# Thealexbarney/VGAudio

Measured on AMD Instinct MI355X. Metric: Msamples/s encoded (GC-ADPCM, 4096 ch) at 1/2/4/8 GPUs; % HBM roofline, higher is better.
Workload: dtype int32; 1 GPU; BASELINE configs[1]: 4096 mono channels x 48 kHz x 60 s GC-ADPCM coefficient search + encode per GPU; parallelism=units sharded x1, channels_per_gpu=4096, samples_per_channel=2880000, bit_exact_channels_checked=0

## Files before the change

vgaudio_amd/csrc/capi_gcadpcm.hip:

```cpp
#include "gc_capi.hpp"
#include "../../include/vgaudio_hip_testing.h"

using namespace vga;

extern "C" {

int vga_testing_gc_plan_pieces(int cus, int groups, int frames, long long group_frames, int ragged, int *out5)
{
    if (!out5 || cus <= 0 || groups <= 0 || frames <= 0) return -1;
    bool persistent = false;
    gc::Pieces seg;
    const int segments = gc::plan_encode_pieces_on(cus, groups, frames, group_frames, ragged != 0, &persistent, &seg);
    out5[0] = segments;
    out5[1] = seg.big;
    out5[2] = seg.nb;
    out5[3] = seg.small;
    out5[4] = persistent ? 1 : 0;
    return 0;
}

int vga_gcadpcm_nibble_count_to_sample_count(int nibble_count) { return gc::nibble_count_to_sample_count(nibble_count); }
int vga_gcadpcm_sample_count_to_nibble_count(int sample_count) { return gc::sample_count_to_nibble_count(sample_count); }
int vga_gcadpcm_nibble_to_sample(int nibble) { return gc::nibble_to_sample(nibble); }
int vga_gcadpcm_sample_to_nibble(int sample) { return gc::sample_to_nibble(sample); }
int vga_gcadpcm_sample_count_to_byte_count(int sample_count) { return gc::sample_count_to_byte_count(sample_count); }
int vga_gcadpcm_byte_count_to_sample_count(int byte_count) { return gc::byte_count_to_sample_count(byte_count); }

size_t vga_gcadpcm_coefs_workspace_bytes(int nch, int length)
{
    if (nch <= 0 || length < 0) return 0;
    const size_t frames = ((size_t)length + 13) / 14;
    return (size_t)nch * (size_t)vga::gc::coef_record_pitch((int64_t)frames) * 16;
}

int vga_gcadpcm_coefs_device(const int16_t *d_pcm, int64_t pcm_pitch, int nch, int length, int16_t *d_coefs,
// ... 287 lines not shown
```

vgaudio_amd/csrc/gc_capi.hpp:

```cpp
#pragma once
#include "common.hpp"
#include "host_batch.hpp"
#include "gcadpcm_kernels.hpp"
#include "gc_host.hpp"

#include <cstring>
#include <vector>

namespace vga {
namespace gc {

constexpr int GC_MIN_SHARE_CHANNELS = 128;

struct GcBatch {
    Stream st;
    DevBuf pcm, coefs, adpcm, h1, h2, ws, status;
    int64_t pcm_pitch = 0, adpcm_pitch = 0;
};

inline int upload_hist(DevBuf &d_h1, DevBuf &d_h2, int nch, const int16_t *h1, const int16_t *h2, const Stream *async_on)
{
    DevBuf *const dst[2] = {&d_h1, &d_h2};
    const int16_t *const src[2] = {h1, h2};
    for (int k = 0; k < 2; k++) {
// ... 13 lines not shown
    int64_t records = 0;
    Pieces seg;
    int segments = 1;
    bool persistent = false;
    std::vector<uint32_t> items;

    void build(const int *lengths, int n, int64_t pcm_base, int64_t adpcm_base)
    {
        lay_out(lengths, n, pcm_base, adpcm_base);
        rec_off.resize(n);
        records = 0;
        for (int c = 0; c < n; c++) {
            rec_off[c] = records;
            records += coef_record_pitch(((int64_t)length[c] + 13) / 14);
        }
        items.clear();
        solo_channels = solo_usable = 0;
        if (n > 0 && !uniform && max_length > 0) {
            std::vector<int> by_length(n);
            for (int i = 0; i < n; i++) by_length[i] = length[order[i]];
            solo_channels = ragged_solo_count(by_length.data(), n, total_frames, device_cu_count(), &solo_usable);
            const int groups = (int)group_frames.size();
            const int64_t work = std::accumulate(group_frames.begin(), group_frames.end(), (int64_t)0);
            segments = plan_encode_pieces(groups, (max_length + 13) / 14, work, true, &persistent, &seg);
            if (persistent && groups < (1 << 20) && segments <= 4096) {
                struct Item { int size, y, g; };
                std::vector<Item> list;
                for (int y = 0; y < segments; y++)
                    for (int g = 0; g < groups; g++)
                        if (seg.first(y) < group_frames[g])
                            list.push_back({(int)std::min<int64_t>(seg.frames(y), group_frames[g] - seg.first(y)), y, g});
                std::stable_sort(list.begin(), list.end(), [](const Item &a, const Item &b) { return a.size > b.size; });
                items.reserve(list.size());
                for (const Item &it : list) items.push_back(((uint32_t)it.y << 20) | (uint32_t)it.g);
            } else
                persistent = false;
        }
    }
    size_t table_bytes() const { return (size_t)round_up((int64_t)count * 8, 16) + (size_t)count * 24 + items.size() * 4; }
    void write_tables(unsigned char *host) const
    {
        int *o = reinterpret_cast<int *>(host);
        int *l = o + count;
        int64_t *p = reinterpret_cast<int64_t *>(host + round_up((int64_t)count * 8, 16));
        for (int c = 0; c < count; c++) {
            o[c] = order[c];
            l[c] = length[c];
// ... 58 lines not shown
```

vgaudio_amd/csrc/gc_encode_kernel.hip:

```cpp
#include "common.hpp"
#include "gc_encode_core.hpp"
#include "gcadpcm_kernels.hpp"
#include "seams.hpp"

#include <cstdio>
#include <cstdlib>

namespace vga {
namespace gc {

constexpr int DPP_QUAD_XOR1 = 0xB1;
constexpr int DPP_QUAD_XOR2 = 0x4E;
constexpr int DPP_ROW_HALF_MIRROR = 0x141;
constexpr int DPP_ROW_MIRROR = 0x140;

template <int CTRL>
__device__ __forceinline__ int dpp(int v)
{
    return __builtin_amdgcn_update_dpp(0, v, CTRL, 0xF, 0xF, true);
}

__device__ __forceinline__ unsigned umin32(unsigned a, unsigned b) { return a < b ? a : b; }

template <class Op>
__device__ __forceinline__ unsigned row16_reduce(unsigned v, Op op)
{
// ... 19 lines not shown
    if (out8 && hipMemcpyFromSymbol(out8, HIP_SYMBOL(g_vga_gc_stats), 8 * sizeof(unsigned long long)) != hipSuccess) return -1;
#ifdef VGA_GC_STATS
    if (out8) out8[7] = 1;
#else
    if (out8) out8[7] = 0;
#endif
    if (reset) {
        const unsigned long long zero[8] = {0, 0, 0, 0, 0, 0, 0, 0};
        if (hipMemcpyToSymbol(HIP_SYMBOL(g_vga_gc_stats), zero, sizeof zero) != hipSuccess) return -1;
    }
    return 0;
}
constexpr int SW = 2;
constexpr int ENC_THREADS = 64 * (SW + 1);
#ifndef VGA_GC_ENCODER_PRIO
#define VGA_GC_ENCODER_PRIO 3
#endif
#ifndef VGA_GC_HELPER_PRIO
#define VGA_GC_HELPER_PRIO 0
#endif
#ifndef VGA_GC_PERSISTENT_WAVES_PER_EU
#define VGA_GC_PERSISTENT_WAVES_PER_EU 3, 3
#endif
template <int CPW>
struct Lay {
    static constexpr int CS = CPW * SW;
    static constexpr int TF = 64 / CS;
};
template <int CS, int TF>
struct GcTileT {
    struct Slot {
        uint32_t xw[8];
        int in2048p[16];
        uint32_t pre[8];
        int4 out[4];
    };
    struct Group { Slot f[TF]; uint32_t pad[4]; };
    Group g[CS];
};
typedef short short2v __attribute__((ext_vector_type(2)));
struct XW7 { uint32_t v[7]; };

#define VGA_COLD __device__ __forceinline__

VGA_COLD int prescan_sequential_cold(XW7 xs, uint32_t hist, int c0, int c1)
{
    int x[16];
    unpack_row(xs.v, hist, x);
    return prescan_sequential(x, c0, c1);
}
// ... 56 lines not shown
                if ((unsigned)r.max_overflow > (cap ? 3u : 248u)) {
                    int xg[16];
                    unpack_row(xw, st.hist, xg);
#pragma unroll
                    for (int i = 0; i < 16; i++) VGA_COLD_OPAQUE(xg[i]);
                    r = as_pass_b(resume_passes(xg, st.c0, st.c1, sp - 1, final_sp));
                    sum_exact = 1;
                    break;
                }
                final_sp = sp;
                if (cap || r.max_overflow <= 1) break;
            }
            fin = 1;
        }
    }
    ColdOut o;
    o.r = r;
    o.final_sp = final_sp;
    o.fin = fin;
    o.sum_exact = sum_exact;
    return o;
}

template <bool REPAIR, int CPW, bool RAGGED>
__device__ __forceinline__ void gc_encode_piece(
    const int bx, const int by,
    const int16_t *__restrict__ pcm, int64_t pcm_pitch, int nch, int total_samples, const Pieces seg,
    const int16_t *__restrict__ coefs, const int16_t *__restrict__ hist1,
    const int16_t *__restrict__ hist2, uint8_t *__restrict__ adpcm, int64_t adpcm_pitch, int16_t *__restrict__ seg_state,
    const int *__restrict__ first_open, const Ragged &rg)
{
    constexpr bool repair = REPAIR;
    constexpr int CS = Lay<CPW>::CS, TF = Lay<CPW>::TF;
    using GcTile = GcTileT<CS, TF>;
    int64_t first_frame = seg.first(by);
    int repair_piece = 0;
    if (repair) {
        int k = SEAM_OPEN_LIMIT;
        for (int g = 0; g < CS; g++) {
            const int slot = bx * CS + g;
            if (slot < nch) {
                const int c = RAGGED ? rg.order[slot] : slot;
                k = first_open[c] < k ? first_open[c] : k;
            }
        }
        if (!is_open(k)) return;
        repair_piece = k;
        first_frame = seg.first(k);
    }
    const int total_wg = RAGGED ? rg.length[rg.order[bx * CS]] : total_samples;
    if (first_frame * 14 >= total_wg) return;
    const int64_t piece_samples = repair ? (int64_t)0x7fffffff : (int64_t)seg.frames(by) * 14;
    auto piece_samples_of = [&](int total) {
        const int64_t rem = (int64_t)total - first_frame * 14;
        return (int)(rem < 0 ? 0 : (rem < piece_samples ? rem : piece_samples));
    };
    pcm += first_frame * 14;
    adpcm += first_frame * 8;
    using Slot = typename GcTile::Slot;
    static_assert(TF % 2 == 0, "the frame loop takes a tile's frames in pairs");
    struct Tiles { GcTile t[2]; Slot end; };
    __shared__ Tiles s_tiles;
    GcTile (&s_tile)[2] = s_tiles.t;
    __shared__ int s_ncold[SW];
    const int tid = threadIdx.x;
    const int wave = tid >> 6;
    const bool helper = wave == SW;
    const int lane = tid & 63;
    constexpr int LPC = 64 / CPW;
    int grp = helper ? lane / TF : wave * CPW + lane / LPC;
    const int l16 = lane & (LPC - 1);
    const int hfr = lane % TF;
    const int slot_raw = bx * CS + grp;
    const bool live = slot_raw < nch;
    const int slot = live ? slot_raw : nch - 1;
    const int ch = RAGGED ? rg.order[slot] : slot;
    const int16_t *src = pcm + (RAGGED ? rg.pcm_off[ch] : (int64_t)ch * pcm_pitch);
    uint8_t *dst = adpcm + (RAGGED ? rg.adpcm_off[ch] : (int64_t)ch * adpcm_pitch);

    const int sample_count = piece_samples_of(RAGGED ? rg.length[ch] : total_samples);
    const int full_frames = sample_count / 14;
    const int tail = sample_count - full_frames * 14;
    const int frames = full_frames + (tail ? 1 : 0);
    const int frames_wg = RAGGED ? (piece_samples_of(total_wg) + 13) / 14 : frames;
    const int tiles = (frames_wg + TF - 1) / TF;

    if (helper) {
        __builtin_amdgcn_s_setprio(VGA_GC_HELPER_PRIO);
        uint32_t cpk[8];
#pragma unroll
        for (int p = 0; p < 8; p++)
            cpk[p] = (uint32_t)(uint16_t)coefs[ch * 16 + 2 * p + 1] | ((uint32_t)(uint16_t)coefs[ch * 16 + 2 * p] << 16);
        auto prepare = [&](int tile) {
            const int fr = RAGGED ? imax(imin(tile * TF + hfr, frames - 1), 0) : imin(tile * TF + hfr, frames - 1);
            int in[14];
            uint32_t w[7];
            if (fr < full_frames) {
                const uint32_t *p32 = reinterpret_cast<const uint32_t *>(src + (int64_t)fr * 14);
#pragma unroll
                for (int i = 0; i < 7; i++) w[i] = p32[i];
#pragma unroll
                for (int i = 0; i < 7; i++) {
                    in[2 * i] = (int)(int16_t)(w[i] & 0xFFFF);
                    in[2 * i + 1] = (int)w[i] >> 16;
                }
            } else {
#pragma unroll
                for (int s = 0; s < 14; s++) in[s] = (s < tail) ? (int)src[(int64_t)fr * 14 + s] : 0;
#pragma unroll
                for (int i = 0; i < 7; i++) w[i] = (uint32_t)(in[2 * i] & 0xFFFF) | ((uint32_t)in[2 * i + 1] << 16);
            }
            Slot &T = s_tile[tile & 1].g[grp].f[hfr];
            uint4 *xr = reinterpret_cast<uint4 *>(&T.xw[0]);
            xr[0] = make_uint4(w[0], w[1], w[2], w[3]);
            xr[1] = make_uint4(w[4], w[5], w[6], (!RAGGED || tile * TF + hfr < frames) ? 1u : 0u);
            int4 *qr = reinterpret_cast<int4 *>(&T.in2048p[0]);
            qr[0] = make_int4(pass_b_row(in[0]), pass_b_row(in[1]), pass_b_row(in[2]), pass_b_row(in[3]));
            qr[1] = make_int4(pass_b_row(in[4]), pass_b_row(in[5]), pass_b_row(in[6]), pass_b_row(in[7]));
            qr[2] = make_int4(pass_b_row(in[8]), pass_b_row(in[9]), pass_b_row(in[10]), pass_b_row(in[11]));
            qr[3] = make_int4(pass_b_row(in[12]), pass_b_row(in[13]), 0, 0);
            uint32_t pair[12];
#pragma unroll
            for (int k = 0; k < 12; k++)
                pair[k] = (k & 1) ? __builtin_amdgcn_alignbit(w[(k + 1) / 2], w[(k - 1) / 2], 16) : w[k / 2];
            uint32_t pre[8];
#pragma unroll
            for (int p = 0; p < 8; p++) {
                int dmax = 0, dmin = 0;
#ifdef VGA_GC_ABLATE_HELPER_PRESCAN
                dmax = in[2 + p] & 1023;
                dmin = -(in[3 + p] & 1023);
#else
#pragma unroll
                for (int k = 0; k < 12; k++) {
                    const int predicted = div2048(__builtin_amdgcn_sdot2(__builtin_bit_cast(short2v, pair[k]),
                                                                         __builtin_bit_cast(short2v, cpk[p]), 0, false));
                    const int d = in[k + 2] - predicted;
                    dmax = imax(dmax, d);
                    dmin = imin(dmin, d);
                }
#endif
                pre[p] = (uint32_t)(clamp16i(dmax) & 0xFFFF) | ((uint32_t)clamp16i(dmin) << 16);
            }
            uint4 *pr = reinterpret_cast<uint4 *>(&T.pre[0]);
            pr[0] = make_uint4(pre[0], pre[1], pre[2], pre[3]);
            pr[1] = make_uint4(pre[4], pre[5], pre[6], pre[7]);
        };
        auto flush = [&](int tile) {
            const int fr = tile * TF + hfr;
            if (!live || fr >= frames) return;
            const int4 *rec = &s_tile[tile & 1].g[grp].f[hfr].out[0];
            const int4 r0 = rec[0], r1 = rec[1], r2 = rec[2], r3 = rec[3];
            const int q[14] = {r0.x, r0.y, r0.z, r0.w, r1.x, r1.y, r1.z, r1.w, r2.x, r2.y, r2.z, r2.w, r3.x, r3.y};
            uint2 v;
            pack_frame_mod16(q, r3.z, r3.w, v.x, v.y);
            if (fr < full_frames) {
                *reinterpret_cast<uint2 *>(dst + (int64_t)fr * 8) = v;
            } else {
                const int nbytes = (tail + 2 + 1) / 2;
                const uint64_t both = ((uint64_t)v.y << 32) | v.x;
                for (int b = 0; b < nbytes; b++) dst[(int64_t)fr * 8 + b] = (uint8_t)(both >> (8 * b));
            }
        };
        if (tiles > 0) prepare(0);
        __syncthreads();
        for (int tile = 0; tile < tiles; tile++) {
            if (tile + 1 < tiles) prepare(tile + 1);
            if (tile > 0) flush(tile - 1);
            __syncthreads();
        }
        if (tiles > 0) flush(tiles - 1);
        return;
    }

    __builtin_amdgcn_s_setprio(VGA_GC_ENCODER_PRIO);
    const int wave_u = __builtin_amdgcn_readfirstlane(wave);
    int p = CPW == 4 ? l16 >> 1 : l16;
    const bool cand_b = CPW == 4 && (l16 & 1) != 0;
    const int c0 = coefs[ch * 16 + 2 * p];
    const int c1 = coefs[ch * 16 + 2 * p + 1];
    const bool coef_ok = pass_b_coef_ok(c0, c1);
    int h0 = hist2 ? hist2[ch] : 0;
    int h1 = hist1 ? hist1[ch] : 0;
    if (repair) {
        h0 = seg_state[((int64_t)(repair_piece - 1) * nch + ch) * 2];
        h1 = seg_state[((int64_t)(repair_piece - 1) * nch + ch) * 2 + 1];
    } else if (by > 0 && (!RAGGED || frames > 0)) {
        h0 = src[-2];
        h1 = src[-1];
    }
    uint32_t hpk = pack16(h0, h1);

    if (lane == 0) s_ncold[wave] = 0;
    struct Row { uint32_t xw[7]; int mp[14]; };
    auto read_row = [&](const Slot &T, Row &R) {
        const uint4 *xr = reinterpret_cast<const uint4 *>(&T.xw[0]);
        const uint4 a0 = xr[0], a1 = xr[1];
        asm volatile("" ::"v"(a1.w));
// ... 236 lines not shown
#endif
            st.bump_a = bump_a; st.ov_a = ov_a; st.ov_b = ov_2;
            const ColdOut o = encode_frame_cold(st, r, final_sp, (generic || resume) ? 0 : 1);
            bool sat2 = false;
            int winner = argmin32(o.r, o.fin != 0, sat2);
            if (sat2) {
                uint64_t total = o.r.total;
                if (o.fin != 0 && needs_exact_sum(total, o.sum_exact != 0))
                    total = wide_total(xw, R.mp, o.final_sp);
                winner = argmin64(total, o.fin != 0);
            }
            commit(o.r, o.final_sp, winner);
        } else
            commit(r, final_sp, winner32);
    };
    auto encode_one = [&](Row &R, Slot &S, uint32_t pre) __attribute__((always_inline)) {
        if constexpr (CPW == 4) encode_frame(R, S, pre);
        else encode_frame8(R, S, pre);
    };

#ifdef VGA_DEBUG_TIMESTAMPS
    if (!repair && tid == 0 && gridDim.y != 1) g_vga_enc_ts[2 * ((blockIdx.y * gridDim.x + blockIdx.x) & 32767)] = wall_clock64();
#endif
    __syncthreads();
    for (int tile = 0; tile < tiles; tile++) {
        const int buf = tile & 1;
        const int nf = imin(TF, frames_wg - tile * TF);
#ifndef VGA_GC_NO_TILE_REDERIVE
        {
            unsigned zero = 0;
            asm volatile("" : "+s"(zero));
            const int l = (int)__builtin_amdgcn_mbcnt_hi(~0u, __builtin_amdgcn_mbcnt_lo(~0u, zero));
            grp = wave_u * CPW + l / LPC;
            p = CPW == 4 ? (l & (LPC - 1)) >> 1 : (l & (LPC - 1));
        }
#endif
        Slot *S = &s_tile[buf].g[grp].f[0];
        Row RA, RB;
        read_row(S[0], RA);
#pragma unroll 1
        for (int j = 0; j < nf; j += 2, S += 2) {
            const uint32_t pre_a = read_pre(S[0]);
            read_row(S[1], RB);
            encode_one(RA, S[0], pre_a);
            if (j + 1 < nf) {
                const uint32_t pre_b = read_pre(S[1]);
                read_row(S[2], RA);
                encode_one(RB, S[1], pre_b);
            }
        }
        __syncthreads();
    }
    if (seg_state && !repair && live && l16 == 0) {
        int16_t *st = seg_state + ((int64_t)by * nch + ch) * 2;
        st[0] = (int16_t)pair_lo(hpk);
        st[1] = (int16_t)pair_hi(hpk);
    }
    if (lane == 0) {
        atomicAdd(&g_vga_gc_stats[3], (unsigned long long)frames_wg);
        atomicAdd(&g_vga_gc_stats[4], (unsigned long long)s_ncold[wave]);
        if (wave == 0) atomicAdd(&g_vga_gc_stats[6], 1ull);
    }
#ifdef VGA_DEBUG_TIMESTAMPS
    if (!repair && tid == 0 && gridDim.y != 1) g_vga_enc_ts[2 * ((blockIdx.y * gridDim.x + blockIdx.x) & 32767) + 1] = wall_clock64();
#endif
}


template <bool REPAIR, int CPW, bool RAGGED>
__global__ __launch_bounds__(ENC_THREADS) __attribute__((amdgpu_waves_per_eu(3, 3))) void gc_encode_kernel(
    const int16_t *__restrict__ pcm, int64_t pcm_pitch, int nch, int total_samples, const Pieces seg,
    const int16_t *__restrict__ coefs, const int16_t *__restrict__ hist1,
    const int16_t *__restrict__ hist2, uint8_t *__restrict__ adpcm, int64_t adpcm_pitch, int16_t *__restrict__ seg_state,
    const int *__restrict__ first_open, const Ragged rg)
// ... 302 lines not shown
            auto exists = [&](int piece) { return piece < segments && seg.first(piece) * 14 < total_wg; };
            int at_start = 0, at_end = 0;
            if (exists(y)) {
                if (y >= 1 && atomicAdd(&seam_count[(int64_t)(y - 1) * groups + g], 1) == 1) at_start = y;
                if (exists(y + 1) && atomicAdd(&seam_count[(int64_t)y * groups + g], 1) == 1) at_end = y + 1;
            }
            s_seam[0] = at_start;
            s_seam[1] = at_end;
        }
        __syncthreads();
        const int seam_a = s_seam[0], seam_b = s_seam[1];
        if ((seam_a | seam_b) != 0) {
            __threadfence();
            const int wave = threadIdx.x >> 6, lane = threadIdx.x & 63;
            if (wave < SW) {
                const int slot = g * CS + wave * CPW + (lane >> 3);
                if (seam_a)
                    seam_piece<8>(slot, seam_a, lane, pcm, pcm_pitch, nch, total_samples, seg, coefs, adpcm, adpcm_pitch, seg_state,
                               first_open, seam_flag, seam_end, force_open, rg);
                if (seam_b)
                    seam_piece<8>(slot, seam_b, lane, pcm, pcm_pitch, nch, total_samples, seg, coefs, adpcm, adpcm_pitch, seg_state,
                               first_open, seam_flag, seam_end, force_open, rg);
            }
        }
    }
}

template <int LPC>
__global__ __launch_bounds__(64) void gc_encode_chain_kernel(
    const int16_t *__restrict__ pcm, int64_t pcm_pitch, int nch, int total_samples, const Pieces seg, int segments,
    const int16_t *__restrict__ coefs, uint8_t *__restrict__ adpcm, int64_t adpcm_pitch,
    int16_t *__restrict__ seg_state, int *__restrict__ first_open, const int *__restrict__ seam_flag,
    const int *__restrict__ seam_end, int force_open, const Ragged rg)
{
    const int lane = threadIdx.x;
    const int pr = LPC == 16 ? (lane >> 1) & 7 : lane & 7;
    const bool lead = (lane & (LPC - 1)) == 0;
    const int slot_raw = blockIdx.x * (64 / LPC) + lane / LPC;
    const bool live = slot_raw < nch;
    const int slot = live ? slot_raw : nch - 1;
    const int ch = rg.order ? rg.order[slot] : slot;
    if (rg.order) total_samples = rg.length[ch];
    const int mine = live ? first_open[ch] : SEAM_NONE;
    int kmin = mine;
#pragma unroll
    for (int o = LPC; o < 64; o <<= 1) kmin = imin(kmin, __shfl_xor(kmin, o));
// ... 35 lines not shown
        } else if (flagged) {
            have = true;
            v0 = (int)(int16_t)(ended & 0xFFFF);
            v1 = ended >> 16;
        } else
            have = false;
    }
    if (__any(live && have && total_samples % 14 != 0))
        encode_tail_frame<LPC>(src, dst, c0, c1, coef_ok, pr, total_samples, v0, v1, live && have && total_samples % 14 != 0);
    (void)last_k;
    if (live && lead && frames_run) atomicAdd(&g_vga_gc_stats[2], (unsigned long long)frames_run);
    if (live && lead) first_open[ch] = SEAM_NONE;
}

constexpr int MIN_PIECE_FRAMES = 3584;

constexpr int RAGGED_OVERSUBSCRIPTION = 4;
constexpr int PERSISTENT_MIN_GROUPS_FACTOR = 32;
constexpr int PERSISTENT_SCHEDULE_GROUPS_FACTOR = 8;
constexpr int PERSISTENT_ITEMS_PER_WORKGROUP = 4;
constexpr int PERSISTENT_BIG_ROUNDS = 3;
constexpr int PERSISTENT_SMALL_ROUNDS = 2;
constexpr int PERSISTENT_SMALL_FRAMES = 4096;
constexpr int MAX_PIECES = 1024;

static int persistent_wgs_per_cu()
{
#ifdef VGA_TUNING
    if (const char *e = std::getenv("VGA_HIP_GC_WGS_PER_CU")) return imin(imax(std::atoi(e), 1), 5);
#endif
    return 4;
}

int plan_encode_pieces(int groups, int frames, int64_t group_frames, bool ragged, bool *persistent_out, Pieces *seg_out, int layout)
{
    return plan_encode_pieces_on(device_cu_count(), groups, frames, group_frames, ragged, persistent_out, seg_out, layout);
}

int plan_encode_pieces_on(int cus, int groups, int frames, int64_t group_frames, bool ragged, bool *persistent_out, Pieces *seg_out, int layout)
{
    const int pmode = encoder_persistent_mode();
    const bool persistent = layout != 4 && (pmode == 2 || (pmode == 0 && (ragged || groups * PERSISTENT_MIN_GROUPS_FACTOR >= cus * 4)));
    int segments = cus * 4 / (groups > 0 ? groups : 1);
    if (persistent && (pmode == 2 || ragged)) segments = (cus * 4 * PERSISTENT_ITEMS_PER_WORKGROUP + groups - 1) / groups;
    if (ragged) {
        const int64_t want = (int64_t)cus * 4 * (persistent ? PERSISTENT_ITEMS_PER_WORKGROUP : RAGGED_OVERSUBSCRIPTION);
        int64_t piece = (group_frames + want - 1) / want;
        if (piece < MIN_PIECE_FRAMES) piece = MIN_PIECE_FRAMES;
        segments = (int)((frames + piece - 1) / piece);
    }
    if (segments > frames / MIN_PIECE_FRAMES) segments = frames / MIN_PIECE_FRAMES;
    if (segments < 1) segments = 1;
    if (segments > MAX_PIECES) segments = MAX_PIECES;
    if (encoder_segments_override() > 0) segments = imin(imin(imax(frames / 64, 1), encoder_segments_override()), MAX_PIECES);
    Pieces seg;
    seg.big = (frames + segments - 1) / segments;
    seg.nb = segments;
    seg.small = seg.big;
    if (persistent && encoder_segments_override() <= 0 && frames >= 4 * MIN_PIECE_FRAMES &&
        (ragged || groups * PERSISTENT_SCHEDULE_GROUPS_FACTOR >= cus * 4)) {
        int big_rounds = ragged ? PERSISTENT_BIG_ROUNDS + 1 : PERSISTENT_BIG_ROUNDS, small_rounds = PERSISTENT_SMALL_ROUNDS, small = PERSISTENT_SMALL_FRAMES;
#ifdef VGA_TUNING
        if (const char *e = std::getenv("VGA_HIP_GC_SCHEDULE")) std::sscanf(e, "%d,%d,%d", &big_rounds, &small_rounds, &small);
#endif
        small = imax(small, MIN_PIECE_FRAMES);
        big_rounds = imax(big_rounds, 1);
        const int wgs = cus * persistent_wgs_per_cu();
        const int64_t per_wg = group_frames / wgs + 1;
        int ns = (small_rounds * wgs + groups / 2) / groups;
        if ((int64_t)ns * small > frames / 2) ns = frames / (2 * small);
        int big = (int)imax((int)((per_wg - (int64_t)small_rounds * small) / big_rounds), small);
        int nb = (int)((frames - (int64_t)ns * small + big - 1) / big);
        if (nb < 1) nb = 1;
        if (!ragged) big = (int)((frames - (int64_t)ns * small + nb - 1) / nb);
        if (big < small) big = small;
        seg.big = big;
        seg.nb = nb;
        seg.small = small;
        segments = nb + ns;
        while (segments > 1 && seg.first(segments - 1) >= frames) segments--;
        if (segments > MAX_PIECES) {
            segments = MAX_PIECES;
            seg.big = seg.small = (frames + segments - 1) / segments;
            seg.nb = segments;
            while (segments > 1 && seg.first(segments - 1) >= frames) segments--;
        }
    }
    if (seg.first(segments) < frames) {
        seg.big = seg.small = (frames + segments - 1) / segments;
        seg.nb = segments;
    }
    *persistent_out = persistent;
    *seg_out = seg;
    return segments;
}

template <int CPW, bool RAGGED>
static int launch_encode_layout(const int16_t *d_pcm, int64_t pcm_pitch, int nch, int sample_count, const int16_t *d_coefs,
                                const int16_t *d_hist1, const int16_t *d_hist2, uint8_t *d_adpcm, int64_t adpcm_pitch,
                                hipStream_t stream, void *d_scratch, size_t scratch_bytes, const Ragged &rg)
{
    constexpr int CS = Lay<CPW>::CS;
    if (RAGGED) sample_count = rg.max_length;
    if (nch <= 0 || sample_count <= 0) return VGA_OK;
    const int groups = (nch + CS - 1) / CS;
    const int cus = device_cu_count();
    const int frames = (sample_count + 13) / 14;
    bool persistent = false;
    Pieces seg;
    int segments;
    if (RAGGED && rg.items) {
        persistent = rg.persistent != 0;
        seg = rg.seg;
        segments = rg.segments;
    } else {
        segments = plan_encode_pieces(groups, frames, RAGGED ? rg.total_frames / CS : (int64_t)groups * frames, RAGGED, &persistent, &seg, CPW);
    }
    AsyncBuf scratch;
    int16_t *seg_state = nullptr;
    int *first_open = nullptr, *seam_flag = nullptr, *seam_end = nullptr, *queue = nullptr, *seam_count = nullptr;
    if (segments > 1 || persistent) {
        const size_t state_bytes = segments > 1 ? (size_t)round_up((int64_t)segments * nch * 2 * (int64_t)sizeof(int16_t), 16) : 0;
        const size_t open_bytes = (size_t)round_up((int64_t)nch * (int64_t)sizeof(int), 16);
        const size_t count_bytes = persistent && segments > 1 ? (size_t)round_up((int64_t)(segments - 1) * groups * (int64_t)sizeof(int), 16) : 0;
        const size_t need = 3 * state_bytes + open_bytes + 16 + count_bytes;
        unsigned char *base = static_cast<unsigned char *>(d_scratch);
        if (!base || scratch_bytes < need) {
            VGA_HIP_TRY(scratch.alloc(need, stream));
            base = scratch.as<unsigned char>();
        }
        seam_flag = reinterpret_cast<int *>(base + state_bytes);
        seam_end = reinterpret_cast<int *>(base + 2 * state_bytes);
        first_open = reinterpret_cast<int *>(base + 3 * state_bytes);
        queue = reinterpret_cast<int *>(base + 3 * state_bytes + open_bytes);
        if (segments > 1) {
            seg_state = reinterpret_cast<int16_t *>(base);
            VGA_HIP_TRY(fill_no_open_seams(first_open, nch, stream));
        } else
            seg_state = nullptr;
        seam_count = queue + 4;
        if (persistent) VGA_HIP_TRY(hipMemsetAsync(queue, 0, 16 + count_bytes, stream));
    }
    if (persistent) {
        const int items = RAGGED && rg.items ? rg.n_items : groups * segments;
        const int wgs = imin(items, cus * persistent_wgs_per_cu());
        if constexpr (CPW == 8)
            hipLaunchKernelGGL((gc_encode_persistent_kernel<CPW, RAGGED>), dim3(wgs), dim3(ENC_THREADS), 0, stream, d_pcm, pcm_pitch, nch,
                               sample_count, seg, d_coefs, d_hist1, d_hist2, d_adpcm, adpcm_pitch, seg_state, rg, groups, segments, queue,
                               seam_count, first_open, seam_flag, seam_end, force_open_seams());
    } else
        hipLaunchKernelGGL((gc_encode_kernel<false, CPW, RAGGED>), dim3(groups, segments), dim3(ENC_THREADS), 0, stream, d_pcm, pcm_pitch, nch,
                           sample_count, seg, d_coefs, d_hist1, d_hist2, d_adpcm, adpcm_pitch, seg_state,
                           (const int *)nullptr, rg);
    VGA_HIP_TRY(hipGetLastError());
    if (segments > 1) {
        if (!persistent) {
#ifdef VGA_GC_SEAM16_ALWAYS
            const bool wide = CPW == 4;
#else
            const bool wide = CPW == 4 && nch > 64;
#endif
            if (wide)
                hipLaunchKernelGGL(gc_encode_seam_kernel<16>, dim3((nch + 3) / 4, segments - 1), dim3(64), 0, stream, d_pcm, pcm_pitch, nch,
                                   sample_count, seg, d_coefs, d_adpcm, adpcm_pitch, seg_state, first_open, seam_flag, seam_end,
                                   force_open_seams(), rg);
            else
// ... 2 lines not shown
                                   force_open_seams(), rg);
            VGA_HIP_TRY(hipGetLastError());
        }
#ifdef VGA_GC_SEAM16_ALWAYS
        if (CPW == 4)
#else
        if (CPW == 4 && nch > 64)
#endif
            hipLaunchKernelGGL(gc_encode_chain_kernel<16>, dim3((nch + 3) / 4), dim3(64), 0, stream, d_pcm, pcm_pitch, nch, sample_count,
                               seg, segments, d_coefs, d_adpcm, adpcm_pitch, seg_state, first_open, seam_flag, seam_end,
                               force_open_seams(), rg);
        else
            hipLaunchKernelGGL(gc_encode_chain_kernel<8>, dim3((nch + 7) / 8), dim3(64), 0, stream, d_pcm, pcm_pitch, nch, sample_count,
                               seg, segments, d_coefs, d_adpcm, adpcm_pitch, seg_state, first_open, seam_flag, seam_end,
                               force_open_seams(), rg);
        VGA_HIP_TRY(hipGetLastError());
        hipLaunchKernelGGL((gc_encode_kernel<true, CPW, RAGGED>), dim3(groups, 1), dim3(ENC_THREADS), 0, stream, d_pcm, pcm_pitch, nch, sample_count,
                           seg, d_coefs, d_hist1, d_hist2, d_adpcm, adpcm_pitch, seg_state, (const int *)first_open, rg);
        VGA_HIP_TRY(hipGetLastError());
    }
    return VGA_OK;
}

size_t encode_scratch_bytes(int nch) { return (size_t)(nch > 0 ? nch : 0) * (1024 * 12 + 4 + 256) + 8192; }

int launch_encode(const int16_t *d_pcm, int64_t pcm_pitch, int nch, int sample_count, const int16_t *d_coefs,
                  const int16_t *d_hist1, const int16_t *d_hist2, uint8_t *d_adpcm, int64_t adpcm_pitch,
                  hipStream_t stream, void *d_scratch, size_t scratch_bytes, const Ragged *rg)
{
    if (rg)
        return launch_encode_layout<8, true>(d_pcm, 0, nch, 0, d_coefs, d_hist1, d_hist2, d_adpcm, 0, stream, d_scratch,
                                             scratch_bytes, *rg);
    int layout = encoder_layout();
    if (layout == 0)
        layout = encoder_persistent_mode() != 2 && ((nch + 15) / 16) * PERSISTENT_MIN_GROUPS_FACTOR < device_cu_count() * 4 ? 4 : 8;
    if (layout == 4)
        return launch_encode_layout<4, false>(d_pcm, pcm_pitch, nch, sample_count, d_coefs, d_hist1, d_hist2, d_adpcm, adpcm_pitch, stream,
                                              d_scratch, scratch_bytes, Ragged{});
    return launch_encode_layout<8, false>(d_pcm, pcm_pitch, nch, sample_count, d_coefs, d_hist1, d_hist2, d_adpcm, adpcm_pitch, stream,
                                          d_scratch, scratch_bytes, Ragged{});
}

}
}
```

vgaudio_amd/csrc/gcadpcm_kernels.hpp:

```cpp
#pragma once
#include <hip/hip_runtime.h>
#include <cstdint>

namespace vga {
namespace gc {

struct Pieces {
    int big = 0, nb = 0, small = 0;
    __host__ __device__ int64_t first(int k) const { return (int64_t)(k < nb ? k : nb) * big + (int64_t)(k > nb ? k - nb : 0) * small; }
    __host__ __device__ int frames(int k) const { return k < nb ? big : small; }
};
int plan_encode_pieces(int groups, int frames, int64_t group_frames, bool ragged, bool *persistent, Pieces *seg, int layout = 8);
int plan_encode_pieces_on(int cus, int groups, int frames, int64_t group_frames, bool ragged, bool *persistent, Pieces *seg, int layout = 8);

struct Ragged {
    const uint32_t *items = nullptr;
    int n_items = 0, segments = 0, persistent = 0;
    Pieces seg;
    const int *order = nullptr;
    const int *length = nullptr;
    const int64_t *pcm_off = nullptr;
    const int64_t *adpcm_off = nullptr;
    const int64_t *rec_off = nullptr;
    int solo_channels = 0;
    int solo_usable = 0;
    int max_length = 0;
    int64_t total_frames = 0;
};

constexpr int COEF_RECORD_BLOCK = 256;
__host__ __device__ inline int64_t coef_record_pitch(int64_t frames)
{
    return (frames > 0 ? frames + COEF_RECORD_BLOCK - 1 : COEF_RECORD_BLOCK) / COEF_RECORD_BLOCK * COEF_RECORD_BLOCK;
}
// ... 28 lines not shown
```

vgaudio_amd/csrc/runtime.hip:

```cpp
#include "common.hpp"
#include "host_batch.hpp"
#include "../../include/vgaudio_hip_testing.h"

namespace vga {

static thread_local char g_err[512] = "";
static thread_local bool g_err_pending = false;

void set_error(const char *fmt, ...)
{
    va_list ap;
    va_start(ap, fmt);
    vsnprintf(g_err, sizeof g_err, fmt, ap);
    va_end(ap);
    g_err_pending = true;
}

bool take_error_pending()
{
    const bool was = g_err_pending;
    g_err_pending = false;
    return was;
}

// ... 93 lines not shown
int vga_get_devices(int *devices, int capacity)
{
    std::lock_guard<std::mutex> g(g_devices_mutex);
    for (int i = 0; i < (int)g_devices.size() && i < capacity && devices; i++) devices[i] = g_devices[i];
    return (int)g_devices.size();
}

int vga_set_progress_callback(vga_progress_fn fn, void *user)
{
    g_progress_callback.fn = fn;
    g_progress_callback.user = fn ? user : nullptr;
    return VGA_OK;
}

int vga_testing_force_open_seams_this_thread(int mode)
{
    const int old = g_settings.force_open_seams;
    g_settings.force_open_seams = mode;
    return old;
}
int vga_testing_gc_encoder_layout_this_thread(int channels_per_wave)
{
    const int old = g_settings.encoder_layout;
    if (channels_per_wave == 0 || channels_per_wave == 4 || channels_per_wave == 8) g_settings.encoder_layout = channels_per_wave;
    return old;
}
int vga_testing_gc_coefs_variant_this_thread(int variant)
{
    const int old = g_settings.coefs_variant;
    if (variant >= 0 && variant <= 3) g_settings.coefs_variant = variant;
    return old;
}
int vga_testing_gc_encoder_segments_this_thread(int segments)
{
    const int old = g_settings.encoder_segments;
    g_settings.encoder_segments = segments > 0 ? segments : 0;
    return old;
}
int vga_testing_gc_encoder_persistent_this_thread(int mode)
{
    const int old = g_settings.encoder_persistent;
    g_settings.encoder_persistent = mode >= 0 && mode <= 2 ? mode : 0;
    return old;
}
int vga_testing_hca_frames_per_group_this_thread(int frames)
{
    const int old = g_settings.hca_frames_per_group;
// ... 62 lines not shown
```

Measured before the change: 81950 Msamples/s.

## Add self-served single-wave persistent GC-ADPCM encoder with eight-channel work items

Adds a persistent encode kernel in which each 64-thread workgroup prepares its own tiles (loading PCM, pre-scanning predictor ranges into LDS) instead of relying on a dedicated helper wave. It uses a single LDS buffer with wave-local fences in place of block-wide barriers, and it prefetches the next tile's samples while encoding the current one. Work is split into eight-channel groups pulled from an atomic queue, with more workgroups per CU and its own piece-schedule rounds. This path becomes the default for large uniform or ragged workloads. The change is meant to remove barrier and helper-wave overhead and to raise occupancy, at the cost of helper/encoder overlap, extra seam bookkeeping and more scratch memory.

```diff
diff --git a/vgaudio_amd/csrc/capi_gcadpcm.hip b/vgaudio_amd/csrc/capi_gcadpcm.hip
--- a/vgaudio_amd/csrc/capi_gcadpcm.hip
+++ b/vgaudio_amd/csrc/capi_gcadpcm.hip
@@ -10,7 +10,8 @@
     if (!out5 || cus <= 0 || groups <= 0 || frames <= 0) return -1;
     bool persistent = false;
     gc::Pieces seg;
-    const int segments = gc::plan_encode_pieces_on(cus, groups, frames, group_frames, ragged != 0, &persistent, &seg);
+    const int segments = gc::plan_encode_pieces_on(cus, groups, frames, group_frames, ragged != 0, &persistent, &seg,
+                                                     encoder_layout() == 1 ? 1 : 8);
     out5[0] = segments;
     out5[1] = seg.big;
     out5[2] = seg.nb;
diff --git a/vgaudio_amd/csrc/gc_capi.hpp b/vgaudio_amd/csrc/gc_capi.hpp
--- a/vgaudio_amd/csrc/gc_capi.hpp
+++ b/vgaudio_amd/csrc/gc_capi.hpp
@@ -59,7 +59,7 @@
             solo_channels = ragged_solo_count(by_length.data(), n, total_frames, device_cu_count(), &solo_usable);
             const int groups = (int)group_frames.size();
             const int64_t work = std::accumulate(group_frames.begin(), group_frames.end(), (int64_t)0);
-            segments = plan_encode_pieces(groups, (max_length + 13) / 14, work, true, &persistent, &seg);
+            segments = plan_encode_pieces(groups, (max_length + 13) / 14, work, true, &persistent, &seg, encoder_plan_layout(groups, true));
             if (persistent && groups < (1 << 20) && segments <= 4096) {
                 struct Item { int size, y, g; };
                 std::vector<Item> list;
diff --git a/vgaudio_amd/csrc/gc_encode_kernel.hip b/vgaudio_amd/csrc/gc_encode_kernel.hip
--- a/vgaudio_amd/csrc/gc_encode_kernel.hip
+++ b/vgaudio_amd/csrc/gc_encode_kernel.hip
@@ -2,6 +2,7 @@
 #include "gc_encode_core.hpp"
 #include "gcadpcm_kernels.hpp"
 #include "seams.hpp"
+#include "gc_plan8.hpp"
 
 #include <cstdio>
 #include <cstdlib>
@@ -67,10 +68,14 @@
 #ifndef VGA_GC_PERSISTENT_WAVES_PER_EU
 #define VGA_GC_PERSISTENT_WAVES_PER_EU 3, 3
 #endif
-template <int CPW>
+template <int CPW, bool SELF = false>
 struct Lay {
-    static constexpr int CS = CPW * SW;
+    static_assert(!SELF || CPW == 8, "the self-served shape is the (channel, predictor) layout");
+    static constexpr int EW = SELF ? 1 : SW;
+    static constexpr int CS = CPW * EW;
     static constexpr int TF = 64 / CS;
+    static constexpr int THREADS = SELF ? 64 : ENC_THREADS;
+    static constexpr int BUFS = SELF ? 1 : 2;
 };
 template <int CS, int TF>
 struct GcTileT {
@@ -173,7 +178,7 @@
     return o;
 }
 
-template <bool REPAIR, int CPW, bool RAGGED>
+template <bool REPAIR, int CPW, bool RAGGED, bool SELF = false>
 __device__ __forceinline__ void gc_encode_piece(
     const int bx, const int by,
     const int16_t *__restrict__ pcm, int64_t pcm_pitch, int nch, int total_samples, const Pieces seg,
@@ -182,7 +187,8 @@
     const int *__restrict__ first_open, const Ragged &rg)
 {
     constexpr bool repair = REPAIR;
-    constexpr int CS = Lay<CPW>::CS, TF = Lay<CPW>::TF;
+    constexpr int CS = Lay<CPW, SELF>::CS, TF = Lay<CPW, SELF>::TF, BUFS = Lay<CPW, SELF>::BUFS;
+    static_assert(!(SELF && REPAIR), "the repair launch keeps the 2 + 1 shape");
     using GcTile = GcTileT<CS, TF>;
     int64_t first_frame = seg.first(by);
     int repair_piece = 0;
@@ -210,13 +216,13 @@
     adpcm += first_frame * 8;
     using Slot = typename GcTile::Slot;
     static_assert(TF % 2 == 0, "the frame loop takes a tile's frames in pairs");
-    struct Tiles { GcTile t[2]; Slot end; };
+    struct Tiles { GcTile t[BUFS]; Slot end; };
     __shared__ Tiles s_tiles;
-    GcTile (&s_tile)[2] = s_tiles.t;
-    __shared__ int s_ncold[SW];
+    GcTile (&s_tile)[BUFS] = s_tiles.t;
+    __shared__ int s_ncold[Lay<CPW, SELF>::EW];
     const int tid = threadIdx.x;
-    const int wave = tid >> 6;
-    const bool helper = wave == SW;
+    const int wave = SELF ? 0 : tid >> 6;
+    const bool helper = !SELF && wave == SW;
     const int lane = tid & 63;
     constexpr int LPC = 64 / CPW;
     int grp = helper ? lane / TF : wave * CPW + lane / LPC;
@@ -236,6 +242,77 @@
     const int frames_wg = RAGGED ? (piece_samples_of(total_wg) + 13) / 14 : frames;
     const int tiles = (frames_wg + TF - 1) / TF;
 
+    auto load_frame = [&](int tile, uint32_t (&w)[7], int (&in)[14]) __attribute__((always_inline)) {
+        const int fr = RAGGED ? imax(imin(tile * TF + hfr, frames - 1), 0) : imin(tile * TF + hfr, frames - 1);
+        if (fr < full_frames) {
+            const uint32_t *p32 = reinterpret_cast<const uint32_t *>(src + (int64_t)fr * 14);
+#pragma unroll
+            for (int i = 0; i < 7; i++) w[i] = p32[i];
+#pragma unroll
+            for (int i = 0; i < 7; i++) {
+                in[2 * i] = (int)(int16_t)(w[i] & 0xFFFF);
+                in[2 * i + 1] = (int)w[i] >> 16;
+            }
+        } else {
+#pragma unroll
+            for (int s = 0; s < 14; s++) in[s] = (s < tail) ? (int)src[(int64_t)fr * 14 + s] : 0;
+#pragma unroll
+            for (int i = 0; i < 7; i++) w[i] = (uint32_t)(in[2 * i] & 0xFFFF) | ((uint32_t)in[2 * i + 1] << 16);
+        }
+    };
+    auto prepare_from = [&](int tile, const uint32_t (&w)[7], const int (&in)[14], const uint32_t (&cpk)[8]) __attribute__((always_inline)) {
+        Slot &T = s_tile[tile & (BUFS - 1)].g[grp].f[hfr];
+        uint4 *xr = reinterpret_cast<uint4 *>(&T.xw[0]);
+        xr[0] = make_uint4(w[0], w[1], w[2], w[3]);
+        xr[1] = make_uint4(w[4], w[5], w[6], (!RAGGED || tile * TF + hfr < frames) ? 1u : 0u);
+        int4 *qr = reinterpret_cast<int4 *>(&T.in2048p[0]);
+        qr[0] = make_int4(pass_b_row(in[0]), pass_b_row(in[1]), pass_b_row(in[2]), pass_b_row(in[3]));
+        qr[1] = make_int4(pass_b_row(in[4]), pass_b_row(in[5]), pass_b_row(in[6]), pass_b_row(in[7]));
+        qr[2] = make_int4(pass_b_row(in[8]), pass_b_row(in[9]), pass_b_row(in[10]), pass_b_row(in[11]));
+        qr[3] = make_int4(pass_b_row(in[12]), pass_b_row(in[13]), 0, 0);
+        uint32_t pair[12];
+#pragma unroll
+        for (int k = 0; k < 12; k++)
+            pair[k] = (k & 1) ? __builtin_amdgcn_alignbit(w[(k + 1) / 2], w[(k - 1) / 2], 16) : w[k / 2];
+        uint32_t pre[8];
+#pragma unroll
+        for (int p = 0; p < 8; p++) {
+            int dmax = 0, dmin = 0;
+#ifdef VGA_GC_ABLATE_HELPER_PRESCAN
+            dmax = in[2 + p] & 1023;
+            dmin = -(in[3 + p] & 1023);
+#else
+#pragma unroll
+            for (int k = 0; k < 12; k++) {
+                const int predicted = div2048(__builtin_amdgcn_sdot2(__builtin_bit_cast(short2v, pair[k]),
+                                                                     __builtin_bit_cast(short2v, cpk[p]), 0, false));
+                const int d = in[k + 2] - predicted;
+                dmax = imax(dmax, d);
+                dmin = imin(dmin, d);
+            }
+#endif
+            pre[p] = (uint32_t)(clamp16i(dmax) & 0xFFFF) | ((uint32_t)clamp16i(dmin) << 16);
+        }
+        uint4 *pr = reinterpret_cast<uint4 *>(&T.pre[0]);
+        pr[0] = make_uint4(pre[0], pre[1], pre[2], pre[3]);
+        pr[1] = make_uint4(pre[4], pre[5], pre[6], pre[7]);
+    };
+    auto flush = [&](int tile) __attribute__((always_inline)) {
+        const int fr = tile * TF + hfr;
+        if (!live || fr >= frames) return;
+        const int4 *rec = &s_tile[tile & (BUFS - 1)].g[grp].f[hfr].out[0];
+        const int4 r0 = rec[0], r1 = rec[1], r2 = rec[2], r3 = rec[3];
+        const int q[14] = {r0.x, r0.y, r0.z, r0.w, r1.x, r1.y, r1.z, r1.w, r2.x, r2.y, r2.z, r2.w, r3.x, r3.y};
+        uint2 v;
+        pack_frame_mod16(q, r3.z, r3.w, v.x, v.y);
+        if (fr < full_frames) {
+            *reinterpret_cast<uint2 *>(dst + (int64_t)fr * 8) = v;
+        } else {
+            const int nbytes = (tail + 2 + 1) / 2;
+            const uint64_t both = ((uint64_t)v.y << 32) | v.x;
+            for (int b = 0; b < nbytes; b++) dst[(int64_t)fr * 8 + b] = (uint8_t)(both >> (8 * b));
+        }
+    };
     if (helper) {
         __builtin_amdgcn_s_setprio(VGA_GC_HELPER_PRIO);
         uint32_t cpk[8];
@@ -243,75 +320,10 @@
         for (int p = 0; p < 8; p++)
             cpk[p] = (uint32_t)(uint16_t)coefs[ch * 16 + 2 * p + 1] | ((uint32_t)(uint16_t)coefs[ch * 16 + 2 * p] << 16);
         auto prepare = [&](int tile) {
-            const int fr = RAGGED ? imax(imin(tile * TF + hfr, frames - 1), 0) : imin(tile * TF + hfr, frames - 1);
+            uint32_t w[7];
             int in[14];
-            uint32_t w[7];
-            if (fr < full_frames) {
-                const uint32_t *p32 = reinterpret_cast<const uint32_t *>(src + (int64_t)fr * 14);
-#pragma unroll
-                for (int i = 0; i < 7; i++) w[i] = p32[i];
-#pragma unroll
-                for (int i = 0; i < 7; i++) {
-                    in[2 * i] = (int)(int16_t)(w[i] & 0xFFFF);
-                    in[2 * i + 1] = (int)w[i] >> 16;
-                }
-            } else {
-#pragma unroll
-                for (int s = 0; s < 14; s++) in[s] = (s < tail) ? (int)src[(int64_t)fr * 14 + s] : 0;
-#pragma unroll
-                for (int i = 0; i < 7; i++) w[i] = (uint32_t)(in[2 * i] & 0xFFFF) | ((uint32_t)in[2 * i + 1] << 16);
-            }
-            Slot &T = s_tile[tile & 1].g[grp].f[hfr];
-            uint4 *xr = reinterpret_cast<uint4 *>(&T.xw[0]);
-            xr[0] = make_uint4(w[0], w[1], w[2], w[3]);
-            xr[1] = make_uint4(w[4], w[5], w[6], (!RAGGED || tile * TF + hfr < frames) ? 1u : 0u);
-            int4 *qr = reinterpret_cast<int4 *>(&T.in2048p[0]);
-            qr[0] = make_int4(pass_b_row(in[0]), pass_b_row(in[1]), pass_b_row(in[2]), pass_b_row(in[3]));
-            qr[1] = make_int4(pass_b_row(in[4]), pass_b_row(in[5]), pass_b_row(in[6]), pass_b_row(in[7]));
-            qr[2] = make_int4(pass_b_row(in[8]), pass_b_row(in[9]), pass_b_row(in[10]), pass_b_row(in[11]));
-            qr[3] = make_int4(pass_b_row(in[12]), pass_b_row(in[13]), 0, 0);
-            uint32_t pair[12];
-#pragma unroll
-            for (int k = 0; k < 12; k++)
-                pair[k] = (k & 1) ? __builtin_amdgcn_alignbit(w[(k + 1) / 2], w[(k - 1) / 2], 16) : w[k / 2];
-            uint32_t pre[8];
-#pragma unroll
-            for (int p = 0; p < 8; p++) {
-                int dmax = 0, dmin = 0;
-#ifdef VGA_GC_ABLATE_HELPER_PRESCAN
-                dmax = in[2 + p] & 1023;
-                dmin = -(in[3 + p] & 1023);
-#else
-#pragma unroll
-                for (int k = 0; k < 12; k++) {
-                    const int predicted = div2048(__builtin_amdgcn_sdot2(__builtin_bit_cast(short2v, pair[k]),
-                                                                         __builtin_bit_cast(short2v, cpk[p]), 0, false));
-                    const int d = in[k + 2] - predicted;
-                    dmax = imax(dmax, d);
-                    dmin = imin(dmin, d);
-                }
-#endif
-                pre[p] = (uint32_t)(clamp16i(dmax) & 0xFFFF) | ((uint32_t)clamp16i(dmin) << 16);
-            }
-            uint4 *pr = reinterpret_cast<uint4 *>(&T.pre[0]);
-            pr[0] = make_uint4(pre[0], pre[1], pre[2], pre[3]);
-            pr[1] = make_uint4(pre[4], pre[5], pre[6], pre[7]);
-        };
-        auto flush = [&](int tile) {
-            const int fr = tile * TF + hfr;
-            if (!live || fr >= frames) return;
-            const int4 *rec = &s_tile[tile & 1].g[grp].f[hfr].out[0];
-            const int4 r0 = rec[0], r1 = rec[1], r2 = rec[2], r3 = rec[3];
-            const int q[14] = {r0.x, r0.y, r0.z, r0.w, r1.x, r1.y, r1.z, r1.w, r2.x, r2.y, r2.z, r2.w, r3.x, r3.y};
-            uint2 v;
-            pack_frame_mod16(q, r3.z, r3.w, v.x, v.y);
-            if (fr < full_frames) {
-                *reinterpret_cast<uint2 *>(dst + (int64_t)fr * 8) = v;
-            } else {
-                const int nbytes = (tail + 2 + 1) / 2;
-                const uint64_t both = ((uint64_t)v.y << 32) | v.x;
-                for (int b = 0; b < nbytes; b++) dst[(int64_t)fr * 8 + b] = (uint8_t)(both >> (8 * b));
-            }
+            load_frame(tile, w, in);
+            prepare_from(tile, w, in, cpk);
         };
         if (tiles > 0) prepare(0);
         __syncthreads();
@@ -324,7 +336,7 @@
         return;
     }
 
-    __builtin_amdgcn_s_setprio(VGA_GC_ENCODER_PRIO);
+    if constexpr (!SELF) __builtin_amdgcn_s_setprio(VGA_GC_ENCODER_PRIO);
     const int wave_u = __builtin_amdgcn_readfirstlane(wave);
     int p = CPW == 4 ? l16 >> 1 : l16;
     const bool cand_b = CPW == 4 && (l16 & 1) != 0;
@@ -607,9 +619,8 @@
 #ifdef VGA_DEBUG_TIMESTAMPS
     if (!repair && tid == 0 && gridDim.y != 1) g_vga_enc_ts[2 * ((blockIdx.y * gridDim.x + blockIdx.x) & 32767)] = wall_clock64();
 #endif
-    __syncthreads();
-    for (int tile = 0; tile < tiles; tile++) {
-        const int buf = tile & 1;
+    auto encode_tile = [&](int tile) __attribute__((always_inline)) {
+        const int buf = tile & (BUFS - 1);
         const int nf = imin(TF, frames_wg - tile * TF);
 #ifndef VGA_GC_NO_TILE_REDERIVE
         {
@@ -634,7 +645,46 @@
                 encode_one(RB, S[1], pre_b);
             }
         }
+    };
+    if constexpr (SELF) {
+        auto own_lds_done = [&]() __attribute__((always_inline)) {
+            __builtin_amdgcn_fence(__ATOMIC_ACQ_REL, "wavefront");
+            __builtin_amdgcn_s_waitcnt(0xC07F);
+        };
+        auto prepare_self = [&](int tile, const uint32_t (&w)[7]) __attribute__((always_inline)) {
+            uint32_t cp8[8];
+#pragma unroll
+            for (int q = 0; q < 8; q++) cp8[q] = (uint32_t)__shfl((int)cpk, (lane & 56) | q);
+            int in[14];
+#pragma unroll
+            for (int i = 0; i < 7; i++) {
+                in[2 * i] = (int)(int16_t)(w[i] & 0xFFFF);
+                in[2 * i + 1] = (int)w[i] >> 16;
+            }
+            prepare_from(tile, w, in, cp8);
+        };
+        uint32_t wn[7];
+        int unused[14];
+        if (tiles > 0) {
+            load_frame(0, wn, unused);
+            prepare_self(0, wn);
+            own_lds_done();
+        }
+        for (int tile = 0; tile < tiles; tile++) {
+            const bool more = tile + 1 < tiles;
+            if (more) load_frame(tile + 1, wn, unused);
+            encode_tile(tile);
+            own_lds_done();
+            flush(tile);
+            if (more) prepare_self(tile + 1, wn);
+            own_lds_done();
+        }
+    } else {
+    __syncthreads();
+    for (int tile = 0; tile < tiles; tile++) {
+        encode_tile(tile);
         __syncthreads();
+    }
     }
     if (seg_state && !repair && live && l16 == 0) {
         int16_t *st = seg_state + ((int64_t)by * nch + ch) * 2;
@@ -983,6 +1033,60 @@
                     seam_piece<8>(slot, seam_b, lane, pcm, pcm_pitch, nch, total_samples, seg, coefs, adpcm, adpcm_pitch, seg_state,
                                first_open, seam_flag, seam_end, force_open, rg);
             }
+        }
+    }
+}
+
+template <bool RAGGED>
+__global__ __launch_bounds__(64) __attribute__((amdgpu_waves_per_eu(3, 3))) void gc_encode_self_served_kernel(
+    const int16_t *__restrict__ pcm, int64_t pcm_pitch, int nch, int total_samples, const Pieces seg,
+    const int16_t *__restrict__ coefs, const int16_t *__restrict__ hist1,
+    const int16_t *__restrict__ hist2, uint8_t *adpcm, int64_t adpcm_pitch, int16_t *seg_state,
+    const Ragged rg, int groups, int items, int segments, int *__restrict__ queue, int *__restrict__ seam_count, int *first_open,
+    int *seam_flag, int *seam_end, int force_open)
+{
+    constexpr int CS = PLAN8_SLOTS;
+    static_assert(Lay<8, true>::CS == CS && Lay<8, true>::THREADS == 64, "one wave, eight channel slots");
+    const int lane = threadIdx.x;
+    const uint32_t *host_items = RAGGED ? rg.items : nullptr;
+#ifdef VGA_DEBUG_TIMESTAMPS
+    if (lane == 0) g_vga_enc_ts[2 * (blockIdx.x & 32767)] = wall_clock64();
+#endif
+    for (;;) {
+        int item = 0;
+        if (lane == 0) item = atomicAdd(queue, 1);
+        item = __builtin_amdgcn_readfirstlane(item);
+        if (item >= items) {
+#ifdef VGA_DEBUG_TIMESTAMPS
+            if (lane == 0) g_vga_enc_ts[2 * (blockIdx.x & 32767) + 1] = wall_clock64();
+#endif
+            return;
+        }
+        int g, y;
+        if (!plan8_item(item, groups, nch, host_items, g, y)) continue;
+        gc_encode_piece<false, 8, RAGGED, true>(g, y, pcm, pcm_pitch, nch, total_samples, seg, coefs, hist1, hist2, adpcm, adpcm_pitch,
+                                                seg_state, (const int *)nullptr, rg);
+        if (segments <= 1) continue;
+        __threadfence();
+        int at_start = 0, at_end = 0;
+        if (lane == 0) {
+            const int total_wg = RAGGED ? rg.length[rg.order[g * CS]] : total_samples;
+            auto exists = [&](int piece) { return piece < segments && seg.first(piece) * 14 < total_wg; };
+            if (exists(y)) {
+                if (y >= 1 && atomicAdd(&seam_count[(int64_t)(y - 1) * groups + g], 1) == 1) at_start = y;
+                if (exists(y + 1) && atomicAdd(&seam_count[(int64_t)y * groups + g], 1) == 1) at_end = y + 1;
+            }
+        }
+        const int seam_a = __builtin_amdgcn_readfirstlane(at_start), seam_b = __builtin_amdgcn_readfirstlane(at_end);
+        if ((seam_a | seam_b) != 0) {
+            __threadfence();
+            const int slot = g * CS + (lane >> 3);
+            if (seam_a)
+                seam_piece<8>(slot, seam_a, lane, pcm, pcm_pitch, nch, total_samples, seg, coefs, adpcm, adpcm_pitch, seg_state,
+                           first_open, seam_flag, seam_end, force_open, rg);
+            if (seam_b)
+                seam_piece<8>(slot, seam_b, lane, pcm, pcm_pitch, nch, total_samples, seg, coefs, adpcm, adpcm_pitch, seg_state,
+                           first_open, seam_flag, seam_end, force_open, rg);
         }
     }
 }
@@ -1064,6 +1168,8 @@
 constexpr int PERSISTENT_BIG_ROUNDS = 3;
 constexpr int PERSISTENT_SMALL_ROUNDS = 2;
 constexpr int PERSISTENT_SMALL_FRAMES = 4096;
+constexpr int SELF_SERVED_BIG_ROUNDS = 4;
+constexpr int SELF_SERVED_SMALL_ROUNDS = 1;
 constexpr int MAX_PIECES = 1024;
 
 static int persistent_wgs_per_cu()
@@ -1081,8 +1187,9 @@
 
 int plan_encode_pieces_on(int cus, int groups, int frames, int64_t group_frames, bool ragged, bool *persistent_out, Pieces *seg_out, int layout)
 {
+    const bool self = layout == 1;
     const int pmode = encoder_persistent_mode();
-    const bool persistent = layout != 4 && (pmode == 2 || (pmode == 0 && (ragged || groups * PERSISTENT_MIN_GROUPS_FACTOR >= cus * 4)));
+    const bool persistent = self || (layout != 4 && (pmode == 2 || (pmode == 0 && (ragged || groups * PERSISTENT_MIN_GROUPS_FACTOR >= cus * 4))));
     int segments = cus * 4 / (groups > 0 ? groups : 1);
     if (persistent && (pmode == 2 || ragged)) segments = (cus * 4 * PERSISTENT_ITEMS_PER_WORKGROUP + groups - 1) / groups;
     if (ragged) {
@@ -1102,14 +1209,16 @@
     if (persistent && encoder_segments_override() <= 0 && frames >= 4 * MIN_PIECE_FRAMES &&
         (ragged || groups * PERSISTENT_SCHEDULE_GROUPS_FACTOR >= cus * 4)) {
         int big_rounds = ragged ? PERSISTENT_BIG_ROUNDS + 1 : PERSISTENT_BIG_ROUNDS, small_rounds = PERSISTENT_SMALL_ROUNDS, small = PERSISTENT_SMALL_FRAMES;
+        if (self && !ragged) { big_rounds = SELF_SERVED_BIG_ROUNDS; small_rounds = SELF_SERVED_SMALL_ROUNDS; }
 #ifdef VGA_TUNING
         if (const char *e = std::getenv("VGA_HIP_GC_SCHEDULE")) std::sscanf(e, "%d,%d,%d", &big_rounds, &small_rounds, &small);
 #endif
         small = imax(small, MIN_PIECE_FRAMES);
         big_rounds = imax(big_rounds, 1);
-        const int wgs = cus * persistent_wgs_per_cu();
-        const int64_t per_wg = group_frames / wgs + 1;
-        int ns = (small_rounds * wgs + groups / 2) / groups;
+        const int wgs = cus * (self ? PLAN8_WGS_PER_CU : persistent_wgs_per_cu());
+        const int queue_groups = self ? 2 * groups : groups;
+        const int64_t per_wg = group_frames * (self ? 2 : 1) / wgs + 1;
+        int ns = (small_rounds * wgs + queue_groups / 2) / queue_groups;
         if ((int64_t)ns * small > frames / 2) ns = frames / (2 * small);
         int big = (int)imax((int)((per_wg - (int64_t)small_rounds * small) / big_rounds), small);
         int nb = (int)((frames - (int64_t)ns * small + big - 1) / big);
@@ -1137,6 +1246,17 @@
     return segments;
 }
 
+#ifndef VGA_GC_SELF_SERVED_DEFAULT
+#define VGA_GC_SELF_SERVED_DEFAULT 1
+#endif
+static bool self_served_shape(int layout_hook, int groups16, int cus, bool ragged)
+{
+    if (layout_hook == 1) return true;
+    if (layout_hook != 0 || encoder_persistent_mode() != 0) return false;
+    return VGA_GC_SELF_SERVED_DEFAULT != 0 && (ragged || groups16 * PERSISTENT_SCHEDULE_GROUPS_FACTOR >= cus * 4);
+}
+int encoder_plan_layout(int groups16, bool ragged) { return self_served_shape(encoder_layout(), groups16, device_cu_count(), ragged) ? 1 : 8; }
+
 template <int CPW, bool RAGGED>
 static int launch_encode_layout(const int16_t *d_pcm, int64_t pcm_pitch, int nch, int sample_count, const int16_t *d_coefs,
                                 const int16_t *d_hist1, const int16_t *d_hist2, uint8_t *d_adpcm, int64_t adpcm_pitch,
@@ -1151,20 +1271,25 @@
     bool persistent = false;
     Pieces seg;
     int segments;
+    const bool want_self = CPW == 8 && self_served_shape(encoder_layout(), groups, cus, RAGGED);
     if (RAGGED && rg.items) {
         persistent = rg.persistent != 0;
         seg = rg.seg;
         segments = rg.segments;
     } else {
-        segments = plan_encode_pieces(groups, frames, RAGGED ? rg.total_frames / CS : (int64_t)groups * frames, RAGGED, &persistent, &seg, CPW);
-    }
+        segments = plan_encode_pieces(groups, frames, RAGGED ? rg.total_frames / CS : (int64_t)groups * frames, RAGGED, &persistent, &seg,
+                                      want_self ? 1 : CPW);
+    }
+    const bool self = want_self && persistent;
+    const Plan8 p8 = self ? plan_groups_of_eight(cus, nch, segments, RAGGED && rg.items ? rg.n_items : -1) : Plan8{};
+    const int seam_groups = self ? p8.groups : groups;
     AsyncBuf scratch;
     int16_t *seg_state = nullptr;
     int *first_open = nullptr, *seam_flag = nullptr, *seam_end = nullptr, *queue = nullptr, *seam_count = nullptr;
     if (segments > 1 || persistent) {
         const size_t state_bytes = segments > 1 ? (size_t)round_up((int64_t)segments * nch * 2 * (int64_t)sizeof(int16_t), 16) : 0;
         const size_t open_bytes = (size_t)round_up((int64_t)nch * (int64_t)sizeof(int), 16);
-        const size_t count_bytes = persistent && segments > 1 ? (size_t)round_up((int64_t)(segments - 1) * groups * (int64_t)sizeof(int), 16) : 0;
+        const size_t count_bytes = persistent && segments > 1 ? (size_t)round_up((int64_t)(segments - 1) * seam_groups * (int64_t)sizeof(int), 16) : 0;
         const size_t need = 3 * state_bytes + open_bytes + 16 + count_bytes;
         unsigned char *base = static_cast<unsigned char *>(d_scratch);
         if (!base || scratch_bytes < need) {
@@ -1183,7 +1308,12 @@
         seam_count = queue + 4;
         if (persistent) VGA_HIP_TRY(hipMemsetAsync(queue, 0, 16 + count_bytes, stream));
     }
-    if (persistent) {
+    if (self) {
+        if constexpr (CPW == 8)
+            hipLaunchKernelGGL((gc_encode_self_served_kernel<RAGGED>), dim3(p8.wgs), dim3(Lay<8, true>::THREADS), 0, stream, d_pcm, pcm_pitch,
+                               nch, sample_count, seg, d_coefs, d_hist1, d_hist2, d_adpcm, adpcm_pitch, seg_state, rg, p8.groups, p8.items,
+                               segments, queue, seam_count, first_open, seam_flag, seam_end, force_open_seams());
+    } else if (persistent) {
         const int items = RAGGED && rg.items ? rg.n_items : groups * segments;
         const int wgs = imin(items, cus * persistent_wgs_per_cu());
         if constexpr (CPW == 8)
@@ -1232,7 +1362,7 @@
     return VGA_OK;
 }
 
-size_t encode_scratch_bytes(int nch) { return (size_t)(nch > 0 ? nch : 0) * (1024 * 12 + 4 + 256) + 8192; }
+size_t encode_scratch_bytes(int nch) { return (size_t)(nch > 0 ? nch : 0) * (1024 * 12 + 4 + 512) + 8192; }
 
 int launch_encode(const int16_t *d_pcm, int64_t pcm_pitch, int nch, int sample_count, const int16_t *d_coefs,
                   const int16_t *d_hist1, const int16_t *d_hist2, uint8_t *d_adpcm, int64_t adpcm_pitch,
diff --git a/vgaudio_amd/csrc/gc_plan8.hpp b/vgaudio_amd/csrc/gc_plan8.hpp
--- /dev/null
+++ b/vgaudio_amd/csrc/gc_plan8.hpp
@@ -0,0 +1,49 @@
+#pragma once
+#include <cstdint>
+
+#if defined(__HIPCC__)
+#define VGA_PLAN8_HD __host__ __device__
+#else
+#define VGA_PLAN8_HD
+#endif
+
+namespace vga {
+namespace gc {
+
+constexpr int PLAN8_SLOTS = 8;
+constexpr int PLAN8_WGS_PER_CU = 12;
+
+struct Plan8 {
+    int groups = 0;
+    int items = 0;
+    int wgs = 0;
+    int rounds_x16 = 0;
+};
+
+inline Plan8 plan_groups_of_eight(int cus, int nch, int segments, int host_items)
+{
+    Plan8 p;
+    if (nch <= 0 || segments <= 0 || cus <= 0) return p;
+    p.groups = (nch + PLAN8_SLOTS - 1) / PLAN8_SLOTS;
+    p.items = host_items >= 0 ? 2 * host_items : p.groups * segments;
+    const int cap = cus * PLAN8_WGS_PER_CU;
+    p.wgs = p.items < cap ? p.items : cap;
+    p.rounds_x16 = p.wgs > 0 ? (int)(((int64_t)p.items * 16 + p.wgs - 1) / p.wgs) : 0;
+    return p;
+}
+
+VGA_PLAN8_HD inline bool plan8_item(int item, int groups8, int nch, const uint32_t *host_items, int &g, int &y)
+{
+    if (host_items) {
+        const uint32_t v = host_items[item >> 1];
+        g = 2 * (int)(v & 0xFFFFFu) + (item & 1);
+        y = (int)(v >> 20);
+    } else {
+        g = item % groups8;
+        y = item / groups8;
+    }
+    return g * PLAN8_SLOTS < nch;
+}
+
+}
+}
diff --git a/vgaudio_amd/csrc/gcadpcm_kernels.hpp b/vgaudio_amd/csrc/gcadpcm_kernels.hpp
--- a/vgaudio_amd/csrc/gcadpcm_kernels.hpp
+++ b/vgaudio_amd/csrc/gcadpcm_kernels.hpp
@@ -10,6 +10,7 @@
     __host__ __device__ int64_t first(int k) const { return (int64_t)(k < nb ? k : nb) * big + (int64_t)(k > nb ? k - nb : 0) * small; }
     __host__ __device__ int frames(int k) const { return k < nb ? big : small; }
 };
+int encoder_plan_layout(int groups, bool ragged);
 int plan_encode_pieces(int groups, int frames, int64_t group_frames, bool ragged, bool *persistent, Pieces *seg, int layout = 8);
 int plan_encode_pieces_on(int cus, int groups, int frames, int64_t group_frames, bool ragged, bool *persistent, Pieces *seg, int layout = 8);
 
diff --git a/vgaudio_amd/csrc/runtime.hip b/vgaudio_amd/csrc/runtime.hip
--- a/vgaudio_amd/csrc/runtime.hip
+++ b/vgaudio_amd/csrc/runtime.hip
@@ -139,7 +139,8 @@
 int vga_testing_gc_encoder_layout_this_thread(int channels_per_wave)
 {
     const int old = g_settings.encoder_layout;
-    if (channels_per_wave == 0 || channels_per_wave == 4 || channels_per_wave == 8) g_settings.encoder_layout = channels_per_wave;
+    if (channels_per_wave == 0 || channels_per_wave == 1 || channels_per_wave == 4 || channels_per_wave == 8)
+        g_settings.encoder_layout = channels_per_wave;
     return old;
 }
 int vga_testing_gc_coefs_variant_this_thread(int variant)
```

New measurement: 84080 Msamples/s (median of 6 runs). 1.03x the previous value.
